# voidstrike/FPSG

Hardware: AMD Instinct MI355X
Metric: episodes/sec (+ Chamfer-kernel HBM GB/s in roofline.hbm), 2048-pt clouds, 224x224 images; episode = fwd + Chamfer + bwd, step = E episodes + all-reduce + Adam (higher is better)
Workload: dtype f32

## Files before the change

### fpsg_amd/_hip.py

```python
from __future__ import annotations

import ctypes
import os
import threading

import torch

_HERE = os.path.dirname(os.path.abspath(__file__))
LIB_PATH = os.environ.get("FPSG_HIP_LIB") or os.path.join(_HERE, "libfpsg_hip.so")

_c_f32p = ctypes.c_void_p
_c_i32p = ctypes.c_void_p
_c_int = ctypes.c_int
_c_stream = ctypes.c_void_p

SIGNATURES = {
    "fpsg_version": [],
    "fpsg_last_error": [],
    "fpsg_chamfer_fwd": [_c_f32p, _c_f32p, _c_int, _c_int, _c_int,
                         _c_f32p, _c_i32p, _c_f32p, _c_i32p, _c_stream],
    "fpsg_chamfer_bwd": [_c_f32p, _c_f32p, _c_i32p, _c_i32p, _c_f32p, _c_f32p,
                         _c_int, _c_int, _c_int, _c_f32p, _c_f32p, _c_stream],
    "fpsg_chamfer_losses": [_c_f32p, _c_f32p, _c_int, _c_int, _c_int, _c_int, ctypes.c_float, ctypes.c_float, _c_f32p,
                            _c_stream],
# ... 41 lines not shown
    "fpsg_softmin": [_c_f32p, _c_f32p, _c_f32p, _c_int, _c_int, _c_int, ctypes.c_float, _c_f32p, _c_stream],
    "fpsg_sinkhorn_workspace_floats": [_c_int, _c_int, _c_int],
    "fpsg_sinkhorn_divergence": [_c_f32p, _c_f32p, _c_int, _c_int, _c_int, ctypes.c_void_p, _c_int, _c_f32p, _c_f32p,
                                 _c_stream],
    "fpsg_sinkhorn_grad_workspace_floats": [_c_int, _c_int, _c_int],
    "fpsg_sinkhorn_divergence_grad": [_c_f32p, _c_f32p, _c_int, _c_int, _c_int, ctypes.c_void_p, _c_int, _c_f32p, _c_f32p,
                                      _c_f32p, _c_f32p, _c_stream],
    "fpsg_dec1_tiles": [_c_int],
    "fpsg_dec1_fwd": [_c_f32p, _c_f32p, _c_int, _c_int, _c_f32p, _c_f32p, _c_f32p, _c_f32p, _c_f32p, _c_int, _c_int,
                      _c_int, _c_int, _c_int, ctypes.c_float, _c_f32p, _c_f32p, _c_f32p, _c_f32p, _c_stream],
    "fpsg_dec1_bwd": [_c_f32p, _c_f32p, _c_f32p, _c_int, _c_int, _c_f32p, _c_f32p, _c_int, _c_int, _c_int, _c_int,
                      _c_int, _c_f32p, _c_f32p, _c_f32p, _c_f32p, _c_f32p, _c_stream],
    "fpsg_dec1_fwd_ld": [_c_f32p, _c_int, _c_f32p, _c_int, _c_int, _c_f32p, _c_int, _c_f32p, _c_f32p, _c_f32p, _c_f32p, _c_int,
                         _c_int, _c_int, _c_int, _c_int, ctypes.c_float, _c_f32p, _c_int, _c_f32p, _c_f32p, _c_f32p,
                         _c_stream],
    "fpsg_dec1_bwd_ld": [_c_f32p, _c_int, _c_f32p, _c_int, _c_f32p, _c_int, _c_int, _c_f32p, _c_int, _c_f32p, _c_int, _c_int,
                         _c_int, _c_int, _c_int, _c_int, _c_f32p, _c_f32p, _c_f32p, _c_f32p, _c_f32p, _c_stream],
    "fpsg_bn_act_rows_fwd": [_c_f32p, _c_int, ctypes.POINTER(ctypes.c_int), ctypes.POINTER(ctypes.c_int), _c_int,
                             _c_f32p, _c_f32p, _c_f32p, _c_int, ctypes.c_float, _c_int, ctypes.c_float, _c_f32p,
                             _c_f32p, _c_f32p, _c_stream],
    "fpsg_bn_act_rows_bwd": [_c_f32p, _c_int, ctypes.POINTER(ctypes.c_int), ctypes.POINTER(ctypes.c_int), _c_int,
                             _c_f32p, _c_f32p, _c_f32p, _c_int, _c_int, ctypes.c_float, _c_f32p, _c_f32p, _c_f32p,
                             _c_f32p, _c_stream],
    "fpsg_bn_workspace_floats": [_c_int, _c_int, _c_int],
    "fpsg_bn_act_fwd": [_c_f32p, _c_f32p, _c_f32p, _c_f32p, _c_f32p, _c_f32p, ctypes.c_float, _c_int, _c_int, _c_int, _c_int,
                        ctypes.c_float, _c_int, ctypes.c_float, _c_f32p, _c_f32p, _c_f32p, _c_f32p, _c_f32p,
                        _c_stream],
    "fpsg_bn_act_bwd": [_c_f32p, _c_f32p, _c_f32p, _c_f32p, _c_int, _c_int, _c_int, _c_int, _c_int,
                        ctypes.c_float, _c_f32p, _c_f32p, _c_f32p, _c_f32p, _c_f32p, _c_f32p, _c_stream],
    "fpsg_bn_act_bwd_coef": [_c_f32p, _c_f32p, _c_f32p, _c_f32p, _c_int, _c_int, _c_int, _c_int, _c_int, ctypes.c_float,
                             _c_f32p, _c_f32p, _c_f32p, _c_f32p, _c_stream],
    "fpsg_bn_act_bwd_parts": [_c_f32p, _c_f32p, _c_f32p, _c_f32p, _c_int, _c_int, _c_int, _c_int, _c_int,
                        ctypes.c_float, _c_f32p, _c_f32p, _c_f32p, _c_f32p, _c_f32p, _c_f32p, _c_f32p, _c_int, _c_stream],
    "fpsg_bn_pool_workspace_floats": [_c_int, _c_int, _c_int, _c_int],
    "fpsg_bn_act_pool_fwd": [_c_f32p, _c_f32p, _c_f32p, _c_f32p, _c_f32p, _c_f32p, ctypes.c_float, _c_int, _c_int, _c_int, _c_int,
                             _c_int, ctypes.c_float, _c_int, ctypes.c_float, _c_f32p, _c_f32p, _c_f32p, _c_f32p,
                             _c_f32p, _c_f32p, _c_int, _c_stream],
    "fpsg_bn_act_pool_bwd": [_c_f32p, _c_f32p, _c_f32p, _c_f32p, _c_int, _c_int, _c_int, _c_int, _c_int, _c_int,
                             ctypes.c_float, _c_f32p, _c_f32p, _c_f32p, _c_f32p, _c_f32p, _c_f32p, _c_stream],
    "fpsg_bn_max_workspace_floats": [_c_int, _c_int, _c_int],
    "fpsg_bn_max_dz_offset": [_c_int, _c_int, _c_int],
    "fpsg_bn_act_max_fwd": [_c_f32p, _c_f32p, _c_f32p, _c_f32p, _c_f32p, _c_f32p, ctypes.c_float, _c_int, _c_int, _c_int, _c_int,
                            ctypes.c_float, _c_int, ctypes.c_float, _c_f32p, _c_i32p, _c_f32p, _c_f32p, _c_f32p,
                            _c_f32p, _c_stream],
    "fpsg_bn_act_max_bwd": [_c_f32p, _c_f32p, _c_f32p, _c_i32p, _c_f32p, _c_int, _c_int, _c_int, _c_int, _c_int,
                            ctypes.c_float, _c_f32p, _c_f32p, _c_f32p, _c_f32p, _c_f32p, _c_f32p, _c_stream],
    "fpsg_max_bwd_prep": [_c_f32p, _c_f32p, _c_f32p, _c_f32p, _c_f32p, _c_f32p, _c_int, _c_int, _c_int, _c_int, _c_f32p, _c_f32p,
                          _c_f32p, _c_f32p, _c_stream],
    "fpsg_max_bwd_dw": [_c_f32p, _c_f32p, _c_f32p, _c_f32p, _c_f32p, _c_int, _c_int, _c_int, _c_f32p, _c_stream],
    "fpsg_max_bwd_gather": [_c_f32p, _c_f32p, _c_i32p, _c_int, _c_int, _c_int, _c_int, _c_f32p, _c_f32p, _c_stream],
    "fpsg_max_bwd_scatter": [_c_f32p, _c_f32p, _c_f32p, _c_f32p, _c_i32p, _c_f32p, _c_int, _c_int, _c_int, _c_int, _c_f32p,
                             _c_stream],
    "fpsg_max_bwd_scatter_workspace_floats": [_c_int, _c_int, _c_int],
    "fpsg_bn_act_max_bwd_coef": [_c_f32p, _c_f32p, _c_f32p, _c_i32p, _c_f32p, _c_int, _c_int, _c_int, _c_int, _c_int,
                                 ctypes.c_float, _c_f32p, _c_f32p, _c_f32p, _c_f32p, _c_stream],
    "fpsg_wino_input_transform": [_c_int, _c_f32p, _c_int, _c_int, _c_int, _c_int, _c_f32p, ctypes.c_long, _c_stream],
    "fpsg_wino_output_transform": [_c_int, _c_f32p, _c_int, _c_int, _c_int, _c_int, _c_f32p, ctypes.c_long, _c_stream],
    "fpsg_wino_stats_parts": [_c_int, _c_int, _c_int, _c_int],
    "fpsg_wino_output_transform_stats": [_c_int, _c_f32p, _c_int, _c_int, _c_int, _c_int, _c_f32p, _c_f32p, _c_f32p,
                                         ctypes.c_long, _c_stream],
    "fpsg_wino_grad_output_transform": [_c_int, _c_f32p, _c_int, _c_int, _c_int, _c_int, _c_f32p, ctypes.c_long, _c_stream],
    "fpsg_wino_grad_transforms": [_c_int, _c_f32p, _c_int, _c_int, _c_int, _c_int, _c_f32p, _c_f32p, ctypes.c_long, _c_stream],
    "fpsg_wino_filter_transform": [_c_int, _c_f32p, _c_int, _c_int, _c_int, _c_f32p, _c_stream],
    "fpsg_wino_output_transform_bwd_stats": [_c_int, _c_f32p, _c_int, _c_int, _c_int, _c_int, _c_f32p, _c_f32p, _c_f32p,
                                             _c_f32p, _c_f32p, ctypes.c_long, _c_stream],
    "fpsg_wino_filter_transform_batch": [ctypes.c_void_p, _c_int, ctypes.c_long, _c_stream],
    "fpsg_wino_filter_grad_transform": [_c_int, _c_f32p, _c_int, _c_int, _c_f32p, _c_stream],
    "fpsg_wino_conv_fused": [_c_f32p, _c_f32p, _c_int, _c_int, _c_int, _c_int, _c_int, _c_f32p, _c_stream],
    "fpsg_wino_input_transform_act": [_c_int, _c_f32p, _c_f32p, _c_f32p, _c_int, _c_int, _c_int, _c_int, _c_f32p, ctypes.c_long,
                                      _c_stream],
    "fpsg_wino_conv_fused_act": [_c_f32p, _c_f32p, _c_f32p, _c_f32p, _c_int, _c_int, _c_int, _c_int, _c_int, _c_f32p,
                                 _c_stream],
    "fpsg_wino_dw_fused_workspace_floats": [_c_int, _c_int, _c_int, _c_int],
    "fpsg_wino_dw_fused": [_c_f32p, _c_f32p, _c_f32p, _c_f32p, _c_int, _c_int, _c_int, _c_int, _c_int, _c_f32p, _c_f32p,
                           _c_stream],
    "fpsg_wino_conv_fused_parts": [_c_int, _c_int, _c_int, _c_int],
    "fpsg_wino_conv_fused_stats": [_c_f32p, _c_f32p, _c_f32p, _c_f32p, _c_int, _c_int, _c_int, _c_int, _c_int, _c_f32p,
                                   _c_f32p, _c_f32p, _c_stream],
    "fpsg_bn_stats": [_c_f32p, _c_f32p, _c_f32p, _c_f32p, _c_f32p, _c_f32p, ctypes.c_float, _c_int, _c_int, _c_int, _c_int,
                      ctypes.c_float, _c_f32p, _c_f32p, _c_f32p, _c_f32p, _c_f32p, _c_int, _c_stream],
    "fpsg_conv_first_dw_workspace_floats": [_c_int, _c_int, _c_int],
    "fpsg_conv_first_parts": [_c_int, _c_int, _c_int],
    "fpsg_conv_first_fwd": [_c_f32p, _c_f32p, _c_int, _c_int, _c_int, _c_int, _c_int, _c_f32p, _c_f32p, _c_f32p, _c_stream],
    "fpsg_conv_first_dw": [_c_f32p, _c_f32p, _c_int, _c_int, _c_int, _c_int, _c_int, _c_f32p, _c_f32p, _c_stream],
    "fpsg_conv_first_dw_fold": [_c_f32p, _c_f32p, _c_f32p, _c_f32p, _c_f32p, _c_f32p, _c_int, _c_int, _c_int, _c_int, _c_int,
                                _c_f32p, _c_f32p, _c_stream],
    "fpsg_adam_step": [_c_f32p, _c_f32p, _c_f32p, _c_f32p, ctypes.c_size_t, ctypes.c_float, ctypes.c_float,
                       ctypes.c_float, ctypes.c_float, _c_int, ctypes.c_float, _c_stream],
    "fpsg_flat_accumulate_segments": [_c_f32p, ctypes.c_void_p, ctypes.c_void_p, _c_int, ctypes.c_size_t, _c_int, _c_stream],
    "fpsg_flat_accumulate_tables": [_c_f32p, ctypes.c_void_p, ctypes.c_void_p, _c_int, _c_int, ctypes.c_size_t, _c_int,
                                    _c_stream],
    "fpsg_adam_step_segments": [_c_f32p, ctypes.c_void_p, ctypes.c_void_p, _c_int, _c_f32p, _c_f32p, ctypes.c_size_t,
                                ctypes.c_float, ctypes.c_float, ctypes.c_float, ctypes.c_float, _c_int, ctypes.c_float,
                                _c_stream],
    "fpsg_grad_norm_workspace_bytes": [ctypes.c_size_t],
    "fpsg_grad_clip_scale": [_c_f32p, ctypes.c_size_t, ctypes.c_float, ctypes.c_float, ctypes.c_void_p, ctypes.c_size_t,
                             _c_f32p, ctypes.c_void_p, _c_stream],
    "fpsg_grad_clip_scale_segments": [ctypes.c_void_p, ctypes.c_void_p, _c_int, ctypes.c_size_t, ctypes.c_float,
                                      ctypes.c_float, ctypes.c_void_p, ctypes.c_size_t, _c_f32p, ctypes.c_void_p,
                                      _c_stream],
    "fpsg_adam_step_dscale": [_c_f32p, _c_f32p, _c_f32p, _c_f32p, ctypes.c_size_t, ctypes.c_float, ctypes.c_float,
                              ctypes.c_float, ctypes.c_float, _c_int, _c_f32p, _c_stream],
    "fpsg_adam_step_segments_dscale": [_c_f32p, ctypes.c_void_p, ctypes.c_void_p, _c_int, _c_f32p, _c_f32p,
                                       ctypes.c_size_t, ctypes.c_float, ctypes.c_float, ctypes.c_float, ctypes.c_float,
                                       _c_int, _c_f32p, _c_stream],
    "fpsg_adam_step_ema": [_c_f32p, _c_f32p, _c_f32p, _c_f32p, _c_f32p, ctypes.c_size_t, ctypes.c_float, ctypes.c_float,
                           ctypes.c_float, ctypes.c_float, _c_int, ctypes.c_float, _c_f32p, ctypes.c_float, _c_stream],
    "fpsg_adam_step_segments_ema": [_c_f32p, ctypes.c_void_p, ctypes.c_void_p, _c_int, _c_f32p, _c_f32p, _c_f32p,
                                    ctypes.c_size_t, ctypes.c_float, ctypes.c_float, ctypes.c_float, ctypes.c_float,
                                    _c_int, ctypes.c_float, _c_f32p, ctypes.c_float, _c_stream],
    "fpsg_flat_swap": [_c_f32p, _c_f32p, ctypes.c_size_t, _c_stream],
    "fpsg_gemm_split_workspace_floats": [_c_int, _c_int, _c_int, _c_int, _c_int, _c_int],
    "fpsg_gemm_split": [_c_f32p, _c_f32p, _c_f32p, _c_int, _c_int, _c_int, _c_int, _c_int, _c_int, _c_int, ctypes.c_long,
                        ctypes.c_long, ctypes.c_long, _c_int, _c_int, _c_f32p, ctypes.c_size_t, _c_stream],
    "fpsg_gemm_split_packed_a_bytes": [_c_int, _c_int, _c_int, _c_int],
    "fpsg_gemm_split_pack_a": [_c_f32p, _c_int, _c_int, _c_int, _c_int, ctypes.c_long, _c_int, ctypes.c_void_p, _c_stream],
    "fpsg_gemm_split_nn_packed": [ctypes.c_void_p, _c_f32p, _c_f32p, _c_int, _c_int, _c_int, _c_int, _c_int, _c_int,
                                  ctypes.c_long, ctypes.c_long, _c_int, _c_stream],
    "fpsg_gemm_split_nn_persistent": [ctypes.c_void_p, _c_f32p, _c_f32p, _c_int, _c_int, _c_int, _c_int, _c_int, _c_int,
                                      ctypes.c_long, ctypes.c_long, _c_int, _c_stream],
    "fpsg_gemm_f32_nn": [_c_f32p, _c_f32p, _c_f32p, _c_int, _c_int, _c_int, _c_int, _c_int, _c_int, _c_int,
                         ctypes.c_long, ctypes.c_long, ctypes.c_long, _c_int, _c_stream],
    "fpsg_emd_workspace_floats": [_c_int, _c_int, _c_int],
    "fpsg_emd_approx": [_c_f32p, _c_f32p, _c_int, _c_int, _c_int, _c_f32p, _c_f32p, _c_f32p, _c_f32p,
                        _c_stream],
    "fpsg_emd_approx_variant": [_c_f32p, _c_f32p, _c_int, _c_int, _c_int, _c_f32p, _c_f32p, _c_f32p, _c_f32p, _c_int,
                                _c_stream],
    "fpsg_emd_exact_workspace_floats": [_c_int, _c_int],
    "fpsg_emd_exact": [_c_f32p, _c_f32p, _c_int, _c_int, ctypes.c_float, _c_int, _c_f32p, _c_f32p, _c_i32p, _c_i32p,
                       _c_f32p, _c_f32p, _c_f32p, _c_stream],
    "fpsg_chamfer_cross": [_c_f32p, _c_f32p, _c_int, _c_int, _c_int, _c_int, _c_f32p, _c_stream],
    "fpsg_emd_cross_workspace_bytes": [_c_int, _c_int, _c_int],
    "fpsg_emd_cross": [_c_f32p, _c_f32p, _c_int, _c_int, _c_int, ctypes.c_float, _c_int, _c_f32p, _c_f32p, _c_i32p,
                       _c_i32p, ctypes.c_void_p, ctypes.c_size_t, _c_stream],
    "fpsg_occupancy_grid_workspace_bytes": [_c_int, _c_int, _c_int],
    "fpsg_occupancy_grid": [_c_f32p, _c_int, _c_int, _c_int, ctypes.c_float, _c_int, _c_i32p, _c_i32p, _c_i32p, _c_i32p,
                            ctypes.c_void_p, ctypes.c_size_t, _c_stream],
    "fpsg_fps_workspace_bytes": [_c_int, _c_int, _c_int],
    "fpsg_fps": [_c_f32p, _c_int, _c_int, _c_int, _c_i32p, _c_i32p, _c_f32p, ctypes.c_void_p, ctypes.c_size_t, _c_stream],
    "fpsg_dist_profile": [_c_f32p, _c_f32p, _c_int, _c_int, _c_int, _c_f32p, _c_int, _c_i32p, _c_f32p, _c_stream],
    "fpsg_dcd": [_c_f32p, _c_i32p, _c_f32p, _c_i32p, _c_int, _c_int, _c_int, ctypes.c_float, _c_f32p, _c_f32p, _c_i32p,
                 _c_i32p, _c_f32p, _c_f32p, _c_stream],
    "fpsg_repulsion_workspace_bytes": [_c_int, _c_int, _c_int],
    "fpsg_repulsion_fwd": [_c_f32p, _c_int, _c_int, _c_int, ctypes.c_float, _c_i32p, _c_f32p, _c_f32p, ctypes.c_void_p,
                           ctypes.c_size_t, _c_stream],
    "fpsg_repulsion_bwd": [_c_f32p, _c_i32p, _c_f32p, _c_f32p, _c_int, _c_int, _c_int, ctypes.c_float, _c_f32p, _c_stream],
    "fpsg_swd_workspace_bytes": [_c_int, _c_int, _c_int],
    "fpsg_swd": [_c_f32p, _c_f32p, _c_f32p, _c_int, _c_int, _c_int, _c_f32p, _c_f32p, _c_f32p, _c_i32p, _c_i32p,
                 ctypes.c_void_p, ctypes.c_size_t, _c_stream],
}
_RESTYPES = {"fpsg_last_error": ctypes.c_char_p, "fpsg_grad_norm_workspace_bytes": ctypes.c_size_t,
"fpsg_chamfer_workspace_bytes": ctypes.c_size_t,
             "fpsg_sinkhorn_workspace_floats": ctypes.c_size_t,
             "fpsg_sinkhorn_grad_workspace_floats": ctypes.c_size_t,
             "fpsg_knn_workspace_floats": ctypes.c_size_t,
             "fpsg_bn_workspace_floats": ctypes.c_size_t, "fpsg_bn_pool_workspace_floats": ctypes.c_size_t, "fpsg_bn_max_workspace_floats": ctypes.c_size_t, "fpsg_bn_max_dz_offset": ctypes.c_size_t, "fpsg_conv_first_dw_workspace_floats": ctypes.c_size_t, "fpsg_emd_workspace_floats": ctypes.c_size_t, "fpsg_emd_exact_workspace_floats": ctypes.c_size_t, "fpsg_emd_cross_workspace_bytes": ctypes.c_size_t, "fpsg_occupancy_grid_workspace_bytes": ctypes.c_size_t, "fpsg_fps_workspace_bytes": ctypes.c_size_t, "fpsg_max_bwd_scatter_workspace_floats": ctypes.c_size_t,
             "fpsg_wino_dw_fused_workspace_floats": ctypes.c_size_t, "fpsg_gemm_split_workspace_floats": ctypes.c_size_t, "fpsg_gemm_split_packed_a_bytes": ctypes.c_size_t, "fpsg_edgeconv_stats_ws_floats": ctypes.c_size_t,
             "fpsg_repulsion_workspace_bytes": ctypes.c_size_t,
             "fpsg_swd_workspace_bytes": ctypes.c_size_t}

_lib = None
_lock = threading.Lock()


class FpsgHipError(RuntimeError):
    pass
# ... 48 lines not shown
```

### fpsg_amd/csrc/conv_first.hip

```cpp
#include "fpsg_common.h"

namespace fpsg {
namespace {

constexpr int kFirstThreads = 256;

struct FoldArgs {
  const float* y;
  const float* chan;
  const float* coef;
  const float* pre_bias;
};

template <int PX, bool FOLD>
__global__ __launch_bounds__(kFirstThreads) void conv_first_dw_kernel(const float* __restrict__ x,
                                                                      const float* __restrict__ dy, FoldArgs fa, int H, int W,
                                                                      int segs_per_row, int n_segs,
                                                                      float* __restrict__ part ) {
  constexpr int LD = PX + 4;
  constexpr int VPR = PX / 4;
  constexpr int NV = 64 * VPR / kFirstThreads;
  constexpr int PE = 9 * (PX + 2);
  constexpr int NP = (PE + kFirstThreads - 1) / kFirstThreads;
  static_assert(64 * VPR % kFirstThreads == 0, "tile vectors divide over the threads");
// ... 49 lines not shown
        const size_t o = (((size_t)n * 64 + vch[it]) * H + h) * W + w0 + vq4[it];
        rv[it] = *reinterpret_cast<const v4f*>(dy + o);
        if constexpr (FOLD) ry[it] = *reinterpret_cast<const v4f*>(fa.y + o);
      } else if constexpr (FOLD) {
        ry[it] = (v4f){-3.0e38f, -3.0e38f, -3.0e38f, -3.0e38f};
      }
    }
#pragma unroll
    for (int it = 0; it < NP; ++it) {
      const int c = pcr[it] / 3, r = pcr[it] - 3 * c;
      const int hh = h + r - 1, ww = w0 + pj[it] - 1;
      rp[it] = 0.0f;
      if (pcr[it] >= 0 && hh >= 0 && hh < H && ww >= 0 && ww < W) rp[it] = x[(((size_t)n * 3 + c) * H + hh) * W + ww];
    }
  };
  v4f acc[2] = {{0.0f, 0.0f, 0.0f, 0.0f}, {0.0f, 0.0f, 0.0f, 0.0f}};
  int seg = blockIdx.x;
  if (seg < n_segs) fetch(seg);
  for (; seg < n_segs; seg += gridDim.x) {
    __syncthreads();
#pragma unroll
    for (int it = 0; it < NV; ++it) {
      v4f v = rv[it];
      if constexpr (FOLD) {
#pragma unroll
        for (int u = 0; u < 4; ++u) {
          const float xv = ry[it][u] + fb[it];
          const float dz = rv[it][u] * (fma_rn(xv, fsc[it], fsh[it]) > 0.0f ? 1.0f : 0.0f);
          const float dx = fma_rn(fk1[it], dz, fma_rn(fk2[it], xv, fk3[it]));
          v[u] = ry[it][u] == -3.0e38f ? 0.0f : dx;
        }
      }
      *reinterpret_cast<v4f*>(dyt + vch[it] * LD + vq4[it]) = v;
    }
#pragma unroll
    for (int it = 0; it < NP; ++it)
      if (pcr[it] >= 0) xt[pcr[it] * LD + pj[it]] = rp[it];
    __syncthreads();
    if (seg + (int)gridDim.x < n_segs) fetch(seg + gridDim.x);
    const float* ap = dyt + (16 * wave + col) * LD + kk;
    const float* bp0 = xt + boff[0] + kk;
    const float* bp1 = xt + boff[1] + kk;
#pragma unroll
    for (int s = 0; s < PX / 4; ++s) {
      const float a = ap[4 * s];
      const float b0 = bval[0] ? bp0[4 * s] : 0.0f;
      const float b1 = bval[1] ? bp1[4 * s] : 0.0f;
      acc[0] = __builtin_amdgcn_mfma_f32_16x16x4f32(a, b0, acc[0], 0, 0, 0);
      acc[1] = __builtin_amdgcn_mfma_f32_16x16x4f32(a, b1, acc[1], 0, 0, 0);
    }
  }
  float* pp = part + (size_t)blockIdx.x * 64 * 32;
#pragma unroll
  for (int nt = 0; nt < 2; ++nt)
#pragma unroll
    for (int r = 0; r < 4; ++r) pp[(16 * wave + 4 * kk + r) * 32 + 16 * nt + col] = acc[nt][r];
}

__global__ __launch_bounds__(1024) void conv_first_dw_reduce_kernel(const float* __restrict__ part, int n_part,
                                                                    float* __restrict__ dw ) {
  __shared__ double acc[32][32];
  const int k = blockIdx.x, tap = threadIdx.x & 31, g = threadIdx.x >> 5;
  double a = 0.0;
#pragma unroll 8
  for (int p = g; p < n_part; p += 32) a += (double)part[((size_t)p * 64 + k) * 32 + tap];
  acc[g][tap] = a;
  __syncthreads();
  if (g == 0 && tap < 27) {
    double t = acc[0][tap];
#pragma unroll
    for (int q = 1; q < 32; ++q) t += acc[q][tap];
    dw[k * 27 + tap] = (float)t;
  }
}


__device__ __forceinline__ void first_load_weights(const float* __restrict__ wt, const float* __restrict__ bias, int k,
                                                   float (&w)[27], float& b) {
#pragma unroll
  for (int i = 0; i < 27; ++i) w[i] = wt[k * 27 + i];
  b = bias ? bias[k] : 0.0f;
}

__device__ __forceinline__ void first_wait_weights(const float (&w)[27], float b) {
  asm volatile("" ::"s"(w[0]), "s"(w[15]), "s"(w[23]), "s"(w[25]), "s"(w[26]), "s"(b));
  __builtin_amdgcn_sched_barrier(0);
}

__device__ __forceinline__ void first_channel(const float (&d)[3][3][6], const float (&w)[27], float (&o)[4]) {
#pragma unroll
  for (int p = 0; p < 4; ++p) o[p] = 0.0f;
#pragma unroll
  for (int c = 0; c < 3; ++c)
#pragma unroll
    for (int a = 0; a < 3; ++a)
#pragma unroll
      for (int b = 0; b < 3; ++b) {
        const float wv = w[(c * 3 + a) * 3 + b];
#pragma unroll
        for (int p = 0; p < 4; ++p) o[p] = fma_rn(wv, d[c][a][b + p], o[p]);
      }
}

__device__ __forceinline__ void first_lane_sums(const float (&o)[4], float bk, bool live, float& s0, float& s1) {
  s0 = 0.0f;
  s1 = 0.0f;
#pragma unroll
  for (int p = 0; p < 4; ++p) {
    const float v = o[p] + bk;
    s0 += v;
    s1 = fma_rn(v, v, s1);
  }
  if (!live) s0 = s1 = 0.0f;
}

template <bool STATS, bool NT = false>
__global__ __launch_bounds__(kFirstThreads) void conv_first_fwd_kernel(const float* __restrict__ x,
                                                                       const float* __restrict__ wt , int H,
                                                                       int W, long Q, float* __restrict__ y,
                                                                       const float* __restrict__ bias,
                                                                       float* __restrict__ parts) {
  __shared__ float red[kFirstThreads / 64][64][2];
  const int tid = threadIdx.x, lane = tid & 63, wave = tid >> 6;
  const long q_raw = (long)blockIdx.x * kFirstThreads + tid;
  const bool live = q_raw < Q;
  const long q = live ? q_raw : Q - 1;
  const int W4 = W >> 2;
  const int w4 = (int)(q % W4);
  const long t = q / W4;
  const int h = (int)(t % H);
  const long n = t / H;
  const bool has_left = w4 > 0, has_right = w4 < W4 - 1;
  const bool left_lane = has_left && lane > 0, right_lane = has_right && lane < 63;
  v4f mid[3][3];
  float el[3][3], er[3][3];
  const float* rp[3][3];
  bool rin[3];
#pragma unroll
  for (int a = 0; a < 3; ++a) {
    const int r = h + a - 1;
    rin[a] = r >= 0 && r < H;
    const int rc = rin[a] ? r : h;
#pragma unroll
    for (int c = 0; c < 3; ++c) {
      rp[c][a] = x + (((size_t)n * 3 + c) * H + rc) * W + 4 * w4;
      mid[c][a] = *reinterpret_cast<const v4f*>(rp[c][a]);
      el[c][a] = er[c][a] = 0.0f;
    }
  }
  if (has_left && !left_lane) {
#pragma unroll
    for (int a = 0; a < 3; ++a)
#pragma unroll
      for (int c = 0; c < 3; ++c) el[c][a] = rp[c][a][-1];
  }
  if (has_right && !right_lane) {
#pragma unroll
    for (int a = 0; a < 3; ++a)
#pragma unroll
      for (int c = 0; c < 3; ++c) er[c][a] = rp[c][a][4];
  }
  float d[3][3][6];
#pragma unroll
  for (int c = 0; c < 3; ++c) {
#pragma unroll
    for (int a = 0; a < 3; ++a) {
      v4f m = mid[c][a];
      if (!rin[a]) m = (v4f){0.0f, 0.0f, 0.0f, 0.0f};
      float lft = __shfl_up(m[3], 1, 64), rgt = __shfl_down(m[0], 1, 64);
      if (!left_lane) lft = (has_left && rin[a]) ? el[c][a] : 0.0f;
      if (!right_lane) rgt = (has_right && rin[a]) ? er[c][a] : 0.0f;
      d[c][a][0] = lft; d[c][a][1] = m[0]; d[c][a][2] = m[1]; d[c][a][3] = m[2]; d[c][a][4] = m[3]; d[c][a][5] = rgt;
    }
  }
  const size_t plane = (size_t)H * W;
  float* yp = y + ((size_t)n * 64 * H + h) * W + 4 * w4;
  float wa[27], wb[27], ba = 0.0f, bb = 0.0f;
  first_load_weights(wt, STATS ? bias : nullptr, 0, wa, ba);
  for (int k = 0; k < 64; k += 2) {
    first_wait_weights(wa, ba);
    first_load_weights(wt, STATS ? bias : nullptr, k + 1, wb, bb);
    __builtin_amdgcn_sched_barrier(0);
    float oa[4], ob[4];
    first_channel(d, wa, oa);
    if (live) st_stream<NT>(reinterpret_cast<v4f*>(yp + (size_t)k * plane), (v4f){oa[0], oa[1], oa[2], oa[3]});
    float a0 = 0.0f, a1 = 0.0f, b0 = 0.0f, b1 = 0.0f;
    if (STATS) first_lane_sums(oa, ba, live, a0, a1);
    first_wait_weights(wb, bb);
    first_load_weights(wt, STATS ? bias : nullptr, k + 2 < 64 ? k + 2 : 63, wa, ba);
    __builtin_amdgcn_sched_barrier(0);
    first_channel(d, wb, ob);
    if (live) st_stream<NT>(reinterpret_cast<v4f*>(yp + (size_t)(k + 1) * plane), (v4f){ob[0], ob[1], ob[2], ob[3]});
    if (STATS) {
      first_lane_sums(ob, bb, live, b0, b1);
      wave_sum4_to_last(a0, a1, b0, b1);
      if (lane == 63) {
        *reinterpret_cast<v2f*>(&red[wave][k][0]) = (v2f){a0, a1};
        *reinterpret_cast<v2f*>(&red[wave][k + 1][0]) = (v2f){b0, b1};
      }
    }
  }
  if (STATS) {
    __syncthreads();
    if (tid < 64) {
      float t0 = red[0][tid][0], t1 = red[0][tid][1];
#pragma unroll
      for (int w2 = 1; w2 < kFirstThreads / 64; ++w2) { t0 += red[w2][tid][0]; t1 += red[w2][tid][1]; }
      float* out = parts + ((size_t)tid * gridDim.x + blockIdx.x) * 2;
      out[0] = t0;
      out[1] = t1;
    }
  }
}

}
}

extern "C" size_t fpsg_conv_first_dw_workspace_floats(int N, int H, int W) {
  if (N <= 0 || H <= 0 || W <= 0) return 0;
  return (size_t)2048 * 64 * 32;
}

static int conv_first_dw_launch(const char* fn, const float* x, const float* dy, fpsg::FoldArgs fa, int N, int C, int K,
                                int H, int W, float* dw, float* ws, fpsg_stream_t stream) {
  using namespace fpsg;
  const bool fold = fa.y != nullptr;
  FPSG_REQUIRE(C == 3 && K == 64, FPSG_E_SHAPE, "%s: the 3 -> 64 channel layer only (got %d -> %d)", fn, C, K);
  FPSG_REQUIRE(N > 0 && H > 0 && W > 0 && W % 4 == 0, FPSG_E_SHAPE,
               "%s: N, H positive and W a positive multiple of 4 (got %d,%d,%d)", fn, N, H, W);
  FPSG_REQUIRE_PTR(x); FPSG_REQUIRE_PTR(dy); FPSG_REQUIRE_PTR(dw); FPSG_REQUIRE_PTR(ws);
  FPSG_REQUIRE((reinterpret_cast<uintptr_t>(dy) & 15) == 0 && (reinterpret_cast<uintptr_t>(fa.y) & 15) == 0, FPSG_E_ALIGN,
               "%s: dy / y / ga must be 16-byte aligned", fn);
  hipStream_t s = static_cast<hipStream_t>(stream);
  const int px = W % 112 == 0 ? 112 : 64;
  const int segs_per_row = (W + px - 1) / px;
  const long n_segs_l = (long)N * H * segs_per_row;
  FPSG_REQUIRE(n_segs_l < (1L << 31), FPSG_E_LIMIT, "fpsg_conv_first_dw: %ld row segments beyond the 32-bit walk", n_segs_l);
  const int n_segs = (int)n_segs_l;
  const int resident = px == 112 ? 1024 : 2048;
  const int blocks = n_segs < resident ? n_segs : resident;
  if (px == 112 && fold)
    hipLaunchKernelGGL((conv_first_dw_kernel<112, true>), dim3(blocks), dim3(kFirstThreads), 0, s, x, dy, fa, H, W, segs_per_row, n_segs, ws);
  else if (px == 112)
    hipLaunchKernelGGL((conv_first_dw_kernel<112, false>), dim3(blocks), dim3(kFirstThreads), 0, s, x, dy, fa, H, W, segs_per_row, n_segs, ws);
  else if (fold)
    hipLaunchKernelGGL((conv_first_dw_kernel<64, true>), dim3(blocks), dim3(kFirstThreads), 0, s, x, dy, fa, H, W, segs_per_row, n_segs, ws);
  else
    hipLaunchKernelGGL((conv_first_dw_kernel<64, false>), dim3(blocks), dim3(kFirstThreads), 0, s, x, dy, fa, H, W, segs_per_row, n_segs, ws);
  int rc = launch_status(fn);
  if (rc) return rc;
  hipLaunchKernelGGL(conv_first_dw_reduce_kernel, dim3(64), dim3(1024), 0, s, ws, blocks, dw);
  return launch_status(fn);
}

extern "C" int fpsg_conv_first_dw(const float* x, const float* dy, int N, int C, int K, int H, int W, float* dw,
                                  float* ws, fpsg_stream_t stream) {
  return conv_first_dw_launch("fpsg_conv_first_dw", x, dy, fpsg::FoldArgs{nullptr, nullptr, nullptr, nullptr}, N, C, K, H, W,
                              dw, ws, stream);
}

extern "C" int fpsg_conv_first_dw_fold(const float* x, const float* y, const float* ga, const float* chan,
                                       const float* coef, const float* pre_bias, int N, int C, int K, int H, int W,
                                       float* dw, float* ws, fpsg_stream_t stream) {
  using namespace fpsg;
  FPSG_REQUIRE_PTR(y); FPSG_REQUIRE_PTR(chan); FPSG_REQUIRE_PTR(coef);
  FPSG_REQUIRE(!misaligned4(pre_bias), FPSG_E_ALIGN, "fpsg_conv_first_dw_fold: pre_bias not 4-byte aligned");
  return conv_first_dw_launch("fpsg_conv_first_dw_fold", x, ga, FoldArgs{y, chan, coef, pre_bias}, N, C, K, H, W, dw, ws,
                              stream);
}

extern "C" int fpsg_conv_first_parts(int N, int H, int W) {
  if (N <= 0 || H <= 0 || W <= 0 || W % 4) return 0;
  const long Q = (long)N * H * (W / 4);
  return (int)((Q + fpsg::kFirstThreads - 1) / fpsg::kFirstThreads);
}

extern "C" int fpsg_conv_first_fwd(const float* x, const float* w, int N, int C, int K, int H, int W, float* y,
                                   const float* bias, float* parts, fpsg_stream_t stream) {
  using namespace fpsg;
  FPSG_REQUIRE(C == 3 && K == 64, FPSG_E_SHAPE, "fpsg_conv_first_fwd: the 3 -> 64 channel layer only (got %d -> %d)", C, K);
  FPSG_REQUIRE(N > 0 && H > 0 && W > 0 && W % 4 == 0, FPSG_E_SHAPE,
               "fpsg_conv_first_fwd: N, H positive and W a positive multiple of 4 (got %d,%d,%d)", N, H, W);
  FPSG_REQUIRE_PTR(x); FPSG_REQUIRE_PTR(w); FPSG_REQUIRE_PTR(y);
  FPSG_REQUIRE(((reinterpret_cast<uintptr_t>(x) | reinterpret_cast<uintptr_t>(y)) & 15) == 0, FPSG_E_ALIGN,
               "fpsg_conv_first_fwd: x and y must be 16-byte aligned");
  FPSG_REQUIRE(!misaligned4(bias) && !misaligned4(parts) && !misaligned4(w), FPSG_E_ALIGN,
               "fpsg_conv_first_fwd: w / bias / parts not 4-byte aligned");
  const long Q = (long)N * H * (W / 4);
  const long blocks = (Q + kFirstThreads - 1) / kFirstThreads;
  FPSG_REQUIRE(blocks < (1L << 31), FPSG_E_LIMIT, "fpsg_conv_first_fwd: %ld workgroups beyond the grid limit", blocks);
  hipStream_t s = static_cast<hipStream_t>(stream);
  const bool nt = beyond_cache((size_t)N * 64 * H * W * sizeof(float));
  if (parts && nt)
    hipLaunchKernelGGL((conv_first_fwd_kernel<true, true>), dim3((unsigned)blocks), dim3(kFirstThreads), 0, s, x, w, H, W, Q, y, bias, parts);
  else if (parts)
    hipLaunchKernelGGL(conv_first_fwd_kernel<true>, dim3((unsigned)blocks), dim3(kFirstThreads), 0, s, x, w, H, W, Q, y, bias, parts);
  else if (nt)
    hipLaunchKernelGGL((conv_first_fwd_kernel<false, true>), dim3((unsigned)blocks), dim3(kFirstThreads), 0, s, x, w, H, W, Q, y, nullptr, nullptr);
  else
    hipLaunchKernelGGL(conv_first_fwd_kernel<false>, dim3((unsigned)blocks), dim3(kFirstThreads), 0, s, x, w, H, W, Q, y, nullptr, nullptr);
  return launch_status("fpsg_conv_first_fwd");
}
```

### fpsg_amd/winograd.py

```python
from __future__ import annotations

import os

import torch

from . import _hip, gemm_split
from .bn_counters import count_batch

MIN_CHANNELS_M4 = 64
MIN_CHANNELS_M2 = 128
MIN_WIDE_CHANNELS_M2 = 256


def enabled() -> bool:
    return os.environ.get("FPSG_WINOGRAD", "1") != "0"


def _eligible_layer(conv: torch.nn.Conv2d, H: int, W: int) -> bool:
    def is_(v, want):
        return v == want or v == (want, want)
    return (enabled() and is_(conv.kernel_size, 3) and is_(conv.stride, 1) and is_(conv.padding, 1) and is_(conv.dilation, 1)
            and conv.groups == 1 and conv.padding_mode == "zeros" and H % 2 == 0 and W % 2 == 0
            and _wide_enough(conv.in_channels, conv.out_channels, tile_size(H, W)))

# ... 454 lines not shown
            if mode != 2:
                _call("fpsg_bn_stats", _hip.ptr(y), opt(pre_bias), opt(gamma), opt(beta), opt(running_mean), opt(running_var),
                      float(momentum), N, C, H * W, 1 if training else 0, float(eps), _hip.ptr(chan), None, None,
                      opt(ws), _hip.ptr(parts) if use_parts else None, parts.shape[1] if use_parts else 0,
                      _hip.stream_of(y))
            if _can_fuse(m, C, K, N * H * W, H, W):
                if want_parts:
                    out, out_parts = _fused_stats(y, chan, pre_bias, _filter(m, w, False), stats_bias)
                else:
                    out = _fused_act(y, chan, pre_bias, _filter(m, w, False))
                V = None
            else:
                V = _input_act(m, y, chan, pre_bias)
                Mt = _bmm(_filter(m, w, False), V)
                if want_parts:
                    out, out_parts = _output(m, Mt, N, H, W, stats_bias, True)
                else:
                    out = _output(m, Mt, N, H, W)
        ctx.save_for_backward(y, chan, pre_bias, w, V if ctx.needs_input_grad[9] else None)
        ctx.cfg = (N, C, H, W, m, bool(training), gamma is not None, beta is not None)
        if not want_parts:
            return out
        if out_parts is not None:
            ctx.mark_non_differentiable(out_parts)
        return out, out_parts

    @staticmethod
    def backward(ctx, gout, _gparts=None):
        if gout is None:
            return (None,) * 14
        y, chan, pre_bias, w, V = ctx.saved_tensors
        N, C, H, W, m, training, has_g, has_b = ctx.cfg
        K = w.shape[0]
        lib = _hip.load()
        dev = y.device
        gout = gout.contiguous()
        gw = None
        with torch.cuda.device(dev):
            bwd_parts = None
            fuse_dx = _can_fuse(m, K, C, N * H * W, H, W)
            fuse_dw = V is None and _can_fuse_dw(m, C, K, N, H, W)
            Vg = dM = None
            if ctx.needs_input_grad[9] and not fuse_dx and not fuse_dw and grad_transforms_enabled():
                Vg, dM = _grad_transforms(m, gout)
            if fuse_dx:
                ga = _fused(gout, _filter(m, w, True))
            elif bwd_stats_enabled() and N * H * W > _BN_SMALL_MAX:
                ga, bwd_parts = _output_bwd_stats(m, _bmm(_filter(m, w, True), Vg if Vg is not None else _input(m, gout)),
                                                  N, H, W, y, pre_bias, chan)
            else:
                ga = _output(m, _bmm(_filter(m, w, True), Vg if Vg is not None else _input(m, gout)), N, H, W)
            Vg = None
            if ctx.needs_input_grad[9]:
                if fuse_dw:
                    gw = _filter_grad(m, _fused_dw(y, chan, pre_bias, gout), w)
                else:
                    if V is None:
                        V = _input_act(m, y, chan, pre_bias)
                    gw = _filter_grad(m, _bmm_nt(dM if dM is not None else _grad_output(m, gout), V), w)
            want_dpb = pre_bias is not None and ctx.needs_input_grad[1]
            dy = torch.empty_like(y)
            dgamma = torch.empty((C,), dtype=torch.float32, device=dev)
            dbeta = torch.empty((C,), dtype=torch.float32, device=dev)
            dpb = torch.empty((C,), dtype=torch.float32, device=dev) if want_dpb else None
            coef = torch.empty((3, C), dtype=torch.float32, device=dev)
            ws = torch.empty((lib.fpsg_bn_workspace_floats(N, C, H * W),), dtype=torch.float32, device=dev)
            if bwd_parts is not None:
                _call("fpsg_bn_act_bwd_parts", _hip.ptr(y), _hip.ptr(pre_bias) if pre_bias is not None else None,
                      _hip.ptr(ga), _hip.ptr(chan), N, C, H * W, 1 if training else 0, 1, 0.0, _hip.ptr(dy),
                      _hip.ptr(dgamma), _hip.ptr(dbeta), _hip.ptr(dpb) if want_dpb else None, _hip.ptr(coef),
                      _hip.ptr(ws), _hip.ptr(bwd_parts), bwd_parts.shape[1], _hip.stream_of(y))
            else:
                _call("fpsg_bn_act_bwd", _hip.ptr(y), _hip.ptr(pre_bias) if pre_bias is not None else None, _hip.ptr(ga),
                      _hip.ptr(chan), N, C, H * W, 1 if training else 0, 1, 0.0, _hip.ptr(dy), _hip.ptr(dgamma),
                      _hip.ptr(dbeta), _hip.ptr(dpb) if want_dpb else None, _hip.ptr(coef), _hip.ptr(ws), _hip.stream_of(y))
        return (dy, dpb, dgamma if has_g else None, dbeta if has_b else None, None, None, None, None, None, gw, None,
                None, None, None)


def stem_fold_enabled() -> bool:
    return os.environ.get("FPSG_STEM_FOLD", "1") != "0"


class _StemConvBNReluConv(torch.autograd.Function):

    @staticmethod
    def forward(ctx, x, w1, b1, gamma, beta, running_mean, running_var, momentum, eps, w2, m, stats_bias=None,
                want_parts=False):
        from . import conv_first
        ctx.set_materialize_grads(False)
        y1, parts1 = conv_first._forward(x, w1, b1, True)
        N, C, H, W = y1.shape
        K = w2.shape[0]
        lib = _hip.load()
        dev = y1.device
        chan = torch.empty((4, C), dtype=torch.float32, device=dev)
        opt = lambda t: _hip.ptr(t) if t is not None else None
        out_parts = None
        w2c = w2.contiguous()
        with torch.cuda.device(dev):
            _call("fpsg_bn_stats", _hip.ptr(y1), opt(b1), opt(gamma), opt(beta), opt(running_mean), opt(running_var),
                  float(momentum), N, C, H * W, 1, float(eps), _hip.ptr(chan), None, None, None, _hip.ptr(parts1),
                  parts1.shape[1], _hip.stream_of(y1))
            if _can_fuse(m, C, K, N * H * W, H, W):
                if want_parts:
                    out, out_parts = _fused_stats(y1, chan, b1, _filter(m, w2c, False), stats_bias)
                else:
                    out = _fused_act(y1, chan, b1, _filter(m, w2c, False))
                V = None
            else:
                V = _input_act(m, y1, chan, b1)
                Mt = _bmm(_filter(m, w2c, False), V)
                if want_parts:
                    out, out_parts = _output(m, Mt, N, H, W, stats_bias, True)
                else:
                    out = _output(m, Mt, N, H, W)
        ctx.save_for_backward(x, w1, y1, chan, b1, w2c, V if ctx.needs_input_grad[9] else None)
        ctx.cfg = (N, C, H, W, m, gamma is not None, beta is not None)
        if not want_parts:
            return out
        if out_parts is not None:
            ctx.mark_non_differentiable(out_parts)
        return out, out_parts

    @staticmethod
    def backward(ctx, gout, _gparts=None):
        if gout is None:
            return (None,) * 13
        x, w1, y1, chan, b1, w2, V = ctx.saved_tensors
        N, C, H, W, m, has_g, has_b = ctx.cfg
        K = w2.shape[0]
        lib = _hip.load()
        dev = y1.device
        gout = gout.contiguous()
        gw1 = gw2 = db1 = None
        with torch.cuda.device(dev):
            if _can_fuse(m, K, C, N * H * W, H, W):
                ga = _fused(gout, _filter(m, w2, True))
            else:
                ga = _output(m, _bmm(_filter(m, w2, True), _input(m, gout)), N, H, W)
            if ctx.needs_input_grad[9]:
                if V is None and _can_fuse_dw(m, C, K, N, H, W):
                    gw2 = _filter_grad(m, _fused_dw(y1, chan, b1, gout), w2)
                else:
                    if V is None:
                        V = _input_act(m, y1, chan, b1)
                    gw2 = _filter_grad(m, _bmm_nt(_grad_output(m, gout), V), w2)
            dgamma = torch.empty((C,), dtype=torch.float32, device=dev)
            dbeta = torch.empty((C,), dtype=torch.float32, device=dev)
            coef = torch.empty((3, C), dtype=torch.float32, device=dev)
            ws = torch.empty((lib.fpsg_bn_workspace_floats(N, C, H * W),), dtype=torch.float32, device=dev)
            _call("fpsg_bn_act_bwd_coef", _hip.ptr(y1), _hip.ptr(b1), _hip.ptr(ga), _hip.ptr(chan), N, C, H * W, 1, 1, 0.0,
                  _hip.ptr(dgamma), _hip.ptr(dbeta), _hip.ptr(coef), _hip.ptr(ws), _hip.stream_of(y1))
            if ctx.needs_input_grad[1]:
                gw1 = torch.empty_like(w1, memory_format=torch.contiguous_format)
                ws1 = torch.empty((lib.fpsg_conv_first_dw_workspace_floats(N, H, W),), dtype=torch.float32, device=dev)
                xc = x.contiguous()
                _call("fpsg_conv_first_dw_fold", _hip.ptr(xc), _hip.ptr(y1), _hip.ptr(ga), _hip.ptr(chan), _hip.ptr(coef),
                      _hip.ptr(b1), N, 3, 64, H, W, _hip.ptr(gw1), _hip.ptr(ws1), _hip.stream_of(y1))
            if ctx.needs_input_grad[2]:
                db1 = torch.zeros((C,), dtype=torch.float32, device=dev)
        return (None, gw1, db1, dgamma if has_g else None, dbeta if has_b else None, None, None, None, None, gw2, None,
                None, None)


def stem_applies(x, conv1, bn1, conv2) -> bool:
    from . import conv_first
    if not (stem_fold_enabled() and fold_enabled() and bn1.training and bn1.track_running_stats and stats_enabled()):
        return False
    if x.requires_grad or not conv_first.eligible(x, conv1) or os.environ.get("FPSG_CONV_FIRST_FWD", "1") == "0":
        return False
    if conv1.bias is None or conv2.bias is None or x.shape[0] * x.shape[2] * x.shape[3] <= _BN_SMALL_MAX:
        return False
    return (isinstance(conv2, torch.nn.Conv2d) and conv2.in_channels == 64
            and _eligible_layer(conv2, x.shape[2], x.shape[3]))


def stem_conv_bn_relu_conv(x, conv1, bn1, conv2, want_parts=False):
    count_batch(bn1)
    mom = 0.1 if bn1.momentum is None else float(bn1.momentum)
    m = tile_size(x.shape[2], x.shape[3])
    return _StemConvBNReluConv.apply(x.contiguous(), conv1.weight, conv1.bias, bn1.weight, bn1.bias, bn1.running_mean,
                                     bn1.running_var, mom, bn1.eps, conv2.weight, m, conv2.bias, bool(want_parts))


def bn_relu_conv3x3(y, pre_bias, bn, weight, m=None, parts=None, stats_bias=None, want_parts=False):
    if m is None:
        m = tile_size(y.shape[2], y.shape[3])
    training = bn.training
    if training:
        count_batch(bn)
# ... 16 lines not shown
```

### include/fpsg_hip.h

```cpp
#ifndef FPSG_HIP_H
#define FPSG_HIP_H

#include <stddef.h>
#include <stdint.h>

#ifdef __cplusplus
extern "C" {
#endif

typedef void* fpsg_stream_t;

#define FPSG_ABI_VERSION 1

#define FPSG_E_NULL   (-1)
#define FPSG_E_SHAPE  (-2)
#define FPSG_E_ALIGN  (-3)
#define FPSG_E_LIMIT  (-4)

int         fpsg_version(void);
const char* fpsg_last_error(void);

int fpsg_chamfer_fwd(const float* xyz1, const float* xyz2, int B, int N, int M,
                     float* dist1, int32_t* idx1, float* dist2, int32_t* idx2,
                     fpsg_stream_t stream);
// ... 209 lines not shown
                        float* running_mean, float* running_var, float momentum, int N, int C, int L, int training,
                        float eps, int act, float slope, float* out, int32_t* idx, float* chan, float* batch_mean,
                        float* batch_var_unbiased, float* ws, fpsg_stream_t stream);
int fpsg_bn_act_max_bwd(const float* x, const float* pre_bias, const float* gout, const int32_t* idx,
                        const float* chan, int N, int C, int L, int training, int act, float slope, float* dx,
                        float* dgamma, float* dbeta, float* dpre_bias, float* coef, float* ws, fpsg_stream_t stream);
int fpsg_bn_act_max_bwd_coef(const float* x, const float* pre_bias, const float* gout, const int32_t* idx,
                             const float* chan, int N, int C, int L, int training, int act, float slope,
                             float* dgamma, float* dbeta, float* coef, float* ws, fpsg_stream_t stream);

int fpsg_max_bwd_gather(const float* a, const float* dz, const int32_t* idx, int B, int K, int C, int L, float* S,
                        float* spart , fpsg_stream_t stream);
int fpsg_max_bwd_prep(const float* W, const float* coef, const float* pre_bias, const float* mean, const float* dz,
                      const float* spart, int B, int K, int C, int L, float* Wk, float* u, float* dpre_bias, float* s,
                      fpsg_stream_t stream);
int fpsg_max_bwd_dw(const float* S, const float* WG, const float* coef, const float* pre_bias, const float* s, int B,
                    int K, int C, float* dw, fpsg_stream_t stream);
size_t fpsg_max_bwd_scatter_workspace_floats(int B, int C, int L);
int fpsg_max_bwd_scatter(float* da, const float* W, const float* k1, const float* dz, const int32_t* idx, const float* v,
                         int B, int K, int C, int L, float* ws, fpsg_stream_t stream);


int fpsg_wino_input_transform(int m, const float* x, int N, int C, int H, int W, float* V, long ldp,
                              fpsg_stream_t stream);
int fpsg_wino_output_transform(int m, const float* M, int N, int K, int H, int W, float* y, long ldp,
                               fpsg_stream_t stream);
int fpsg_wino_stats_parts(int m, int N, int H, int W);
int fpsg_wino_output_transform_stats(int m, const float* M, int N, int K, int H, int W, float* y, const float* bias,
                                     float* parts, long ldp, fpsg_stream_t stream);
int fpsg_wino_output_transform_bwd_stats(int m, const float* M, int N, int K, int H, int W, float* y,
                                         const float* xpre, const float* pre_bias, const float* chan,
                                         float* parts, long ldp, fpsg_stream_t stream);
int fpsg_wino_grad_output_transform(int m, const float* dy, int N, int K, int H, int W, float* dM, long ldp,
                                    fpsg_stream_t stream);
int fpsg_wino_grad_transforms(int m, const float* dy, int N, int K, int H, int W, float* V, float* dM, long ldp,
                              fpsg_stream_t stream);
int fpsg_wino_filter_transform(int m, const float* w, int K, int C, int flip_transpose, float* U,
                               fpsg_stream_t stream);
int fpsg_wino_filter_transform_batch(const int64_t* jobs, int n_jobs, long total_blocks, fpsg_stream_t stream);
int fpsg_wino_filter_grad_transform(int m, const float* dU, int K, int C, float* dw, fpsg_stream_t stream);

size_t fpsg_gemm_split_workspace_floats(int batch, int M, int N, int K, int transB, int variant);
int fpsg_gemm_split(const float* A, const float* B, float* C, int batch, int M, int N, int K, int lda, int ldb, int ldc,
                    long sA, long sB, long sC, int transB, int variant, float* ws, size_t ws_floats,
                    fpsg_stream_t stream);

size_t fpsg_gemm_split_packed_a_bytes(int batch, int M, int K, int variant);
int fpsg_gemm_split_pack_a(const float* A, int batch, int M, int K, int lda, long sA, int variant, void* Ap,
                           fpsg_stream_t stream);
int fpsg_gemm_split_nn_packed(const void* Ap, const float* B, float* C, int batch, int M, int N, int K, int ldb, int ldc,
                              long sB, long sC, int variant, fpsg_stream_t stream);

int fpsg_gemm_split_nn_persistent(const void* Ap, const float* B, float* C, int batch, int M, int N, int K, int ldb, int ldc,
                                  long sB, long sC, int variant, fpsg_stream_t stream);

int fpsg_gemm_f32_nn(const float* A, const float* B, float* C, int batch, int M, int N, int K, int lda, int ldb, int ldc,
                     long sA, long sB, long sC, int variant, fpsg_stream_t stream);

int fpsg_wino_conv_fused(const float* x, const float* U, int N, int C, int K, int H, int W, float* y,
                         fpsg_stream_t stream);

int fpsg_wino_conv_fused_parts(int N, int K, int H, int W);
int fpsg_wino_conv_fused_stats(const float* x, const float* chan, const float* pre_bias, const float* U, int N, int C,
                               int K, int H, int W, float* y, const float* out_bias, float* parts, fpsg_stream_t stream);

size_t fpsg_wino_dw_fused_workspace_floats(int N, int K, int H, int W);
int fpsg_wino_dw_fused(const float* x, const float* chan, const float* pre_bias, const float* dy, int N, int C, int K,
                       int H, int W, float* dU, float* ws, fpsg_stream_t stream);

int fpsg_wino_input_transform_act(int m, const float* x, const float* chan, const float* pre_bias, int N, int C,
                                  int H, int W, float* V, long ldp, fpsg_stream_t stream);
int fpsg_wino_conv_fused_act(const float* x, const float* chan, const float* pre_bias, const float* U, int N, int C,
                             int K, int H, int W, float* y, fpsg_stream_t stream);

size_t fpsg_conv_first_dw_workspace_floats(int N, int H, int W);
int fpsg_conv_first_dw(const float* x, const float* dy, int N, int C, int K, int H, int W, float* dw, float* ws,
                       fpsg_stream_t stream);
int fpsg_conv_first_dw_fold(const float* x, const float* y, const float* ga, const float* chan, const float* coef,
                            const float* pre_bias, int N, int C, int K, int H, int W, float* dw, float* ws,
                            fpsg_stream_t stream);
int fpsg_conv_first_parts(int N, int H, int W);
int fpsg_conv_first_fwd(const float* x, const float* w, int N, int C, int K, int H, int W, float* y, const float* bias,
                        float* parts, fpsg_stream_t stream);

int fpsg_adam_step(float* param, const float* grad, float* exp_avg, float* exp_avg_sq, size_t n, float lr,
                   float beta1, float beta2, float eps, int step, float grad_scale, fpsg_stream_t stream);
int fpsg_adam_step_segments(float* param, const float* const* grad_ptrs, const long long* seg_off, int nseg,
                            float* exp_avg, float* exp_avg_sq, size_t n, float lr, float beta1, float beta2,
                            float eps, int step, float grad_scale, fpsg_stream_t stream);
int fpsg_flat_accumulate_segments(float* flat, const float* const* grad_ptrs, const long long* seg_off, int nseg,
                                  size_t n, int accumulate, fpsg_stream_t stream);
int fpsg_flat_accumulate_tables(float* flat, const float* const* grad_ptrs, const long long* seg_off, int nseg, int ntab,
                                size_t n, int accumulate, fpsg_stream_t stream);

size_t fpsg_grad_norm_workspace_bytes(size_t n);
int fpsg_grad_clip_scale(const float* grad, size_t n, float grad_scale, float max_norm, void* workspace,
                         size_t workspace_bytes, float* out2, double* stats, fpsg_stream_t stream);
int fpsg_grad_clip_scale_segments(const float* const* grad_ptrs, const long long* seg_off, int nseg, size_t n,
                                  float grad_scale, float max_norm, void* workspace, size_t workspace_bytes, float* out2,
                                  double* stats, fpsg_stream_t stream);
int fpsg_adam_step_dscale(float* param, const float* grad, float* exp_avg, float* exp_avg_sq, size_t n, float lr,
                          float beta1, float beta2, float eps, int step, const float* grad_scale_dev,
                          fpsg_stream_t stream);
int fpsg_adam_step_segments_dscale(float* param, const float* const* grad_ptrs, const long long* seg_off, int nseg,
                                   float* exp_avg, float* exp_avg_sq, size_t n, float lr, float beta1, float beta2,
                                   float eps, int step, const float* grad_scale_dev, fpsg_stream_t stream);

int fpsg_adam_step_ema(float* param, const float* grad, float* exp_avg, float* exp_avg_sq, float* ema, size_t n, float lr,
                       float beta1, float beta2, float eps, int step, float grad_scale, const float* grad_scale_dev,
                       float ema_weight, fpsg_stream_t stream);
int fpsg_adam_step_segments_ema(float* param, const float* const* grad_ptrs, const long long* seg_off, int nseg,
                                float* exp_avg, float* exp_avg_sq, float* ema, size_t n, float lr, float beta1,
                                float beta2, float eps, int step, float grad_scale, const float* grad_scale_dev,
                                float ema_weight, fpsg_stream_t stream);
int fpsg_flat_swap(float* a, float* b, size_t n, fpsg_stream_t stream);

#ifdef __cplusplus
}
#endif
#endif
```

Measured before the change: 45.91.

## Recompute stem conv with fused BN+ReLU to materialize activation once

Adds a stem conv kernel variant that applies bias, batch-norm scale/shift and ReLU in its epilogue. The forward path now recomputes the first convolution after the stats pass to write the activated tensor once. The following Winograd conv then reads plain activations instead of applying BN+ReLU on every tile load. The trade is an extra pass over the cheap 3-channel stem conv plus a full 64-channel activation write and read, in exchange for removing the per-tile activation math from the fused Winograd kernel.

```diff
diff --git a/fpsg_amd/_hip.py b/fpsg_amd/_hip.py
--- a/fpsg_amd/_hip.py
+++ b/fpsg_amd/_hip.py
@@ -147,6 +147,7 @@
     "fpsg_conv_first_dw_workspace_floats": [_c_int, _c_int, _c_int],
     "fpsg_conv_first_parts": [_c_int, _c_int, _c_int],
     "fpsg_conv_first_fwd": [_c_f32p, _c_f32p, _c_int, _c_int, _c_int, _c_int, _c_int, _c_f32p, _c_f32p, _c_f32p, _c_stream],
+    "fpsg_conv_first_fwd_act": [_c_f32p, _c_f32p, _c_f32p, _c_f32p, _c_int, _c_int, _c_int, _c_f32p, _c_stream],
     "fpsg_conv_first_dw": [_c_f32p, _c_f32p, _c_int, _c_int, _c_int, _c_int, _c_int, _c_f32p, _c_f32p, _c_stream],
     "fpsg_conv_first_dw_fold": [_c_f32p, _c_f32p, _c_f32p, _c_f32p, _c_f32p, _c_f32p, _c_int, _c_int, _c_int, _c_int, _c_int,
                                 _c_f32p, _c_f32p, _c_stream],
diff --git a/fpsg_amd/csrc/conv_first.hip b/fpsg_amd/csrc/conv_first.hip
--- a/fpsg_amd/csrc/conv_first.hip
+++ b/fpsg_amd/csrc/conv_first.hip
@@ -155,6 +155,20 @@
   b = bias ? bias[k] : 0.0f;
 }
 
+__device__ __forceinline__ void first_load_coefs(const float* __restrict__ chan, int k, float& sc, float& sh) {
+  sc = chan[k];
+  sh = chan[64 + k];
+}
+
+__device__ __forceinline__ void first_wait_coefs(float sc, float sh) { asm volatile("" ::"s"(sc), "s"(sh)); }
+
+__device__ __forceinline__ void first_apply(float (&o)[4], float b, float sc, float sh) {
+  v4f v = {o[0], o[1], o[2], o[3]};
+  asm("" : "+v"(v));
+#pragma unroll
+  for (int p = 0; p < 4; ++p) o[p] = __builtin_fmaxf(fma_rn(v[p] + b, sc, sh), 0.0f);
+}
+
 __device__ __forceinline__ void first_wait_weights(const float (&w)[27], float b) {
   asm volatile("" ::"s"(w[0]), "s"(w[15]), "s"(w[23]), "s"(w[25]), "s"(w[26]), "s"(b));
   __builtin_amdgcn_sched_barrier(0);
@@ -187,12 +201,15 @@
   if (!live) s0 = s1 = 0.0f;
 }
 
-template <bool STATS, bool NT = false>
+template <bool STATS, bool NT = false, bool APPLY = false>
 __global__ __launch_bounds__(kFirstThreads) void conv_first_fwd_kernel(const float* __restrict__ x,
                                                                        const float* __restrict__ wt , int H,
                                                                        int W, long Q, float* __restrict__ y,
                                                                        const float* __restrict__ bias,
-                                                                       float* __restrict__ parts) {
+                                                                       float* __restrict__ parts,
+                                                                       const float* __restrict__ chan = nullptr) {
+  static_assert(!(STATS && APPLY), "the applying pass produces no sums");
+  constexpr bool BIAS = STATS || APPLY;
   __shared__ float red[kFirstThreads / 64][64][2];
   const int tid = threadIdx.x, lane = tid & 63, wave = tid >> 6;
   const long q_raw = (long)blockIdx.x * kFirstThreads + tid;
@@ -249,20 +266,28 @@
   const size_t plane = (size_t)H * W;
   float* yp = y + ((size_t)n * 64 * H + h) * W + 4 * w4;
   float wa[27], wb[27], ba = 0.0f, bb = 0.0f;
-  first_load_weights(wt, STATS ? bias : nullptr, 0, wa, ba);
+  float sca = 1.0f, sha = 0.0f, scb = 1.0f, shb = 0.0f;
+  first_load_weights(wt, BIAS ? bias : nullptr, 0, wa, ba);
+  if (APPLY) first_load_coefs(chan, 0, sca, sha);
   for (int k = 0; k < 64; k += 2) {
+    if (APPLY) first_wait_coefs(sca, sha);
     first_wait_weights(wa, ba);
-    first_load_weights(wt, STATS ? bias : nullptr, k + 1, wb, bb);
+    first_load_weights(wt, BIAS ? bias : nullptr, k + 1, wb, bb);
+    if (APPLY) first_load_coefs(chan, k + 1, scb, shb);
     __builtin_amdgcn_sched_barrier(0);
     float oa[4], ob[4];
     first_channel(d, wa, oa);
+    if (APPLY) first_apply(oa, ba, sca, sha);
     if (live) st_stream<NT>(reinterpret_cast<v4f*>(yp + (size_t)k * plane), (v4f){oa[0], oa[1], oa[2], oa[3]});
     float a0 = 0.0f, a1 = 0.0f, b0 = 0.0f, b1 = 0.0f;
     if (STATS) first_lane_sums(oa, ba, live, a0, a1);
+    if (APPLY) first_wait_coefs(scb, shb);
     first_wait_weights(wb, bb);
-    first_load_weights(wt, STATS ? bias : nullptr, k + 2 < 64 ? k + 2 : 63, wa, ba);
+    first_load_weights(wt, BIAS ? bias : nullptr, k + 2 < 64 ? k + 2 : 63, wa, ba);
+    if (APPLY) first_load_coefs(chan, k + 2 < 64 ? k + 2 : 63, sca, sha);
     __builtin_amdgcn_sched_barrier(0);
     first_channel(d, wb, ob);
+    if (APPLY) first_apply(ob, bb, scb, shb);
     if (live) st_stream<NT>(reinterpret_cast<v4f*>(yp + (size_t)(k + 1) * plane), (v4f){ob[0], ob[1], ob[2], ob[3]});
     if (STATS) {
       first_lane_sums(ob, bb, live, b0, b1);
@@ -374,3 +399,23 @@
     hipLaunchKernelGGL(conv_first_fwd_kernel<false>, dim3((unsigned)blocks), dim3(kFirstThreads), 0, s, x, w, H, W, Q, y, nullptr, nullptr);
   return launch_status("fpsg_conv_first_fwd");
 }
+
+extern "C" int fpsg_conv_first_fwd_act(const float* x, const float* w, const float* chan, const float* pre_bias, int N,
+                                       int H, int W, float* a, fpsg_stream_t stream) {
+  using namespace fpsg;
+  FPSG_REQUIRE(N > 0 && H > 0 && W > 0 && W % 4 == 0, FPSG_E_SHAPE,
+               "fpsg_conv_first_fwd_act: N, H positive and W a positive multiple of 4 (got %d,%d,%d)", N, H, W);
+  FPSG_REQUIRE_PTR(x); FPSG_REQUIRE_PTR(w); FPSG_REQUIRE_PTR(chan); FPSG_REQUIRE_PTR(a);
+  FPSG_REQUIRE(((reinterpret_cast<uintptr_t>(x) | reinterpret_cast<uintptr_t>(a)) & 15) == 0, FPSG_E_ALIGN,
+               "fpsg_conv_first_fwd_act: x and a must be 16-byte aligned");
+  FPSG_REQUIRE(!misaligned4(pre_bias), FPSG_E_ALIGN, "fpsg_conv_first_fwd_act: pre_bias not 4-byte aligned");
+  const long Q = (long)N * H * (W / 4);
+  const long blocks = (Q + kFirstThreads - 1) / kFirstThreads;
+  FPSG_REQUIRE(blocks < (1L << 31), FPSG_E_LIMIT, "fpsg_conv_first_fwd_act: %ld workgroups beyond the grid limit", blocks);
+  hipStream_t s = static_cast<hipStream_t>(stream);
+  if (beyond_cache((size_t)N * 64 * H * W * sizeof(float)))
+    hipLaunchKernelGGL((conv_first_fwd_kernel<false, true, true>), dim3((unsigned)blocks), dim3(kFirstThreads), 0, s, x, w, H, W, Q, a, pre_bias, nullptr, chan);
+  else
+    hipLaunchKernelGGL((conv_first_fwd_kernel<false, false, true>), dim3((unsigned)blocks), dim3(kFirstThreads), 0, s, x, w, H, W, Q, a, pre_bias, nullptr, chan);
+  return launch_status("fpsg_conv_first_fwd_act");
+}
diff --git a/fpsg_amd/winograd.py b/fpsg_amd/winograd.py
--- a/fpsg_amd/winograd.py
+++ b/fpsg_amd/winograd.py
@@ -560,6 +560,18 @@
     return os.environ.get("FPSG_STEM_FOLD", "1") != "0"
 
 
+def stem_act_once_enabled() -> bool:
+    return os.environ.get("FPSG_STEM_ACT_ONCE", "1") != "0"
+
+
+def _stem_activation(x, w1, chan, b1):
+    N, _, H, W = x.shape
+    a1 = torch.empty((N, 64, H, W), dtype=torch.float32, device=x.device)
+    _call("fpsg_conv_first_fwd_act", _hip.ptr(x), _hip.ptr(w1), _hip.ptr(chan), _hip.ptr(b1) if b1 is not None else None,
+          N, H, W, _hip.ptr(a1), _hip.stream_of(x))
+    return a1
+
+
 class _StemConvBNReluConv(torch.autograd.Function):
 
     @staticmethod
@@ -581,10 +593,18 @@
                   float(momentum), N, C, H * W, 1, float(eps), _hip.ptr(chan), None, None, None, _hip.ptr(parts1),
                   parts1.shape[1], _hip.stream_of(y1))
             if _can_fuse(m, C, K, N * H * W, H, W):
-                if want_parts:
-                    out, out_parts = _fused_stats(y1, chan, b1, _filter(m, w2c, False), stats_bias)
-                else:
-                    out = _fused_act(y1, chan, b1, _filter(m, w2c, False))
+                U = _filter(m, w2c, False)
+                if stem_act_once_enabled():
+                    a1 = _stem_activation(x.contiguous(), w1.contiguous(), chan, b1)
+                    if want_parts:
+                        out, out_parts = _fused_stats(a1, None, None, U, stats_bias)
+                    else:
+                        out = _fused(a1, U)
+                    del a1
+                elif want_parts:
+                    out, out_parts = _fused_stats(y1, chan, b1, U, stats_bias)
+                else:
+                    out = _fused_act(y1, chan, b1, U)
                 V = None
             else:
                 V = _input_act(m, y1, chan, b1)
diff --git a/include/fpsg_hip.h b/include/fpsg_hip.h
--- a/include/fpsg_hip.h
+++ b/include/fpsg_hip.h
@@ -315,6 +315,8 @@
 int fpsg_conv_first_parts(int N, int H, int W);
 int fpsg_conv_first_fwd(const float* x, const float* w, int N, int C, int K, int H, int W, float* y, const float* bias,
                         float* parts, fpsg_stream_t stream);
+int fpsg_conv_first_fwd_act(const float* x, const float* w, const float* chan, const float* pre_bias, int N, int H,
+                            int W, float* a, fpsg_stream_t stream);
 
 int fpsg_adam_step(float* param, const float* grad, float* exp_avg, float* exp_avg_sq, size_t n, float lr,
                    float beta1, float beta2, float eps, int step, float grad_scale, fpsg_stream_t stream);
```

Result: no change. 46.01 (median of 3 runs) (+0.2%).
